# VeeraKarthick609/ImageCaptioner

Measured on NVIDIA B200. Metric: kd_train_samples_per_sec, higher is better.
Workload: dtype bf16

## Files before the change

### imagecaptioner_b200/csrc/api.cu

```cuda
#include <stdlib.h>
#include "gemm.cuh"
#include "loss_kernels.cuh"
#include "decoder_kernels.cuh"
#include "recurrent.cuh"
#include "recur_cluster.cuh"
#include "refine_kernels.cuh"
#include "mha_mma.cuh"
#include "optim_kernels.cuh"

using namespace b2c;

namespace {

constexpr int MAXL = B2C_MAX_LAYERS;
constexpr int COLSUM_RS = 160;

int check_device() {
  static int cached = 1;
  if (cached <= 0) return cached;
  int dev = 0;
  B2C_CUDA(cudaGetDevice(&dev));
  int major = 0;
  B2C_CUDA(cudaDeviceGetAttribute(&major, cudaDevAttrComputeCapabilityMajor, dev));
  if (major != 10) { cached = B2C_EARCH; return set_err(B2C_EARCH, "b2c kernels are built for sm_100a only; device has compute capability major %d", major); }
  cached = 0;
  return 0;
}

struct Carver {
  unsigned char* base; size_t off;
  template <typename U> U* take(size_t n) {
    off = align_up(off, 256);
    U* p = base ? reinterpret_cast<U*>(base + off) : reinterpret_cast<U*>((uintptr_t)0);
    off += n * sizeof(U);
    return p;
  }
};

inline int in_dim(const B2CShape& s, int k) { return k == 0 ? s.E : s.H; }

int check_shape(const B2CShape* s) {
  B2C_CHECK_ARG(s != nullptr, "shape is NULL");
  B2C_CHECK_ARG(s->B > 0 && s->T > 0 && s->S > 0 && s->V > 1, "bad shape B=%d T=%d S=%d V=%d", s->B, s->T, s->S, s->V);
  B2C_CHECK_ARG(s->L >= 1 && s->L <= MAXL, "L=%d outside [1,%d]", s->L, MAXL);
  B2C_CHECK_ARG(s->E > 0 && s->E % 8 == 0 && s->H > 0 && s->H % 8 == 0, "E=%d and H=%d must be positive multiples of 8", s->E, s->H);
  B2C_CHECK_ARG((long)s->B * 4 * s->H < 2147483647L && (long)s->B * s->S * s->E < 2147483647L, "B*4H and B*S*E must stay below 2^31 (32-bit index arithmetic in the per-step kernels)");
  return 0;
}

template <typename T> struct Weights {
  T *Wf, *Wh, *Wce, *Wcc, *W1, *W2, *Wih0, *We; T* Wcat[MAXL]; float* bcat[MAXL]; float* bx;
  T* Wuh;
  void carve(Carver& c, const B2CShape& s) {
    Wf = c.take<T>((size_t)s.E * s.E); Wh = c.take<T>((size_t)s.E * s.H);
// ... 72 lines not shown
  int ncl = cdiv(s.B, 32); if (ncl > mx) ncl = mx;
  if (cdiv(s.B, ncl) > CR_RMAX) return 0;
  return ncl;
}

template <typename T> struct TrainWs {
  Weights<T> w;
  float *P, *u; T *emb, *G0, *o1; T* xh[MAXL]; T* gates[MAXL]; float* c[MAXL];
  T* dgates[MAXL]; float* dxh0; float* dxh[MAXL]; float* dc[MAXL]; T* do1; float* dHext; float* ds; T* du; T* dq; T* dP; float* demb; float* partial;
  float *dWx32, *dWe32; T *dWxT, *dWeT; float* partial_side;
  unsigned int* sync;
  float* EP;
  float* evalp;
  T* G0T;
  float* UR;
  size_t bytes;
  void carve(void* base, const B2CShape& s) {
    Carver c{reinterpret_cast<unsigned char*>(base), 0};
    const size_t B = s.B, Tn = s.T, S = s.S, E = s.E, H = s.H, TB = Tn * B;
    w.carve(c, s);
    P = c.take<float>(B * S * E); emb = c.take<T>(TB * E); u = c.take<float>(TB * E); G0 = c.take<T>(TB * 4 * H); o1 = c.take<T>(TB * E);
    for (int k = 0; k < s.L; ++k) {
      xh[k] = c.take<T>((Tn + 1) * B * (in_dim(s, k) + H));
      gates[k] = c.take<T>(TB * 4 * H);
      this->c[k] = c.take<float>((Tn + 1) * B * H);
    }
    for (int k = 0; k < s.L; ++k) {
      dgates[k] = c.take<T>(TB * 4 * H);
      dxh[k] = k == 0 ? nullptr : c.take<float>(TB * 2 * H);
      dc[k] = c.take<float>(B * H);
    }
    dxh0 = c.take<float>(TB * (E + H));
    do1 = c.take<T>(TB * E); dHext = c.take<float>(TB * H); ds = c.take<float>(TB * S);
    du = c.take<T>(TB * E); dq = c.take<T>(B * H); dP = c.take<T>(B * S * E); demb = c.take<float>(TB * E);
    dWx32 = c.take<float>(4 * H * E); dWe32 = c.take<float>(4 * H * E); dWxT = c.take<T>(4 * H * E); dWeT = c.take<T>(4 * H * E);
    size_t mc = (size_t)s.V; if ((size_t)4 * H > mc) mc = 4 * H; if (E > mc) mc = E;
    partial = c.take<float>((size_t)COLSUM_RS * mc); partial_side = c.take<float>((size_t)COLSUM_RS * mc);
    sync = c.take<unsigned int>(128 + 160 * 32);
    EP = c.take<float>(B * S * E);
    evalp = c.take<float>(TB * (size_t)cdiv(s.V, 32) * EVAL_PART_FLOATS);
    G0T = c.take<T>(cluster_shape_ok(s) ? Tn * (size_t)CR_MAX_CLUSTERS * 4 * H * CR_RMAX : 0);
    UR = c.take<float>(B * (E + 4 * H));
    bytes = align_up(c.off, 256);
  }
};

template <typename T> struct DecodeWs {
  Weights<T> w;
  float *P, *u; T *emb, *G0, *o1; T* xh[MAXL]; float* c[MAXL]; float* logits; int64_t* cur; int32_t* done; float* amax_v; int* amax_i;
  size_t bytes;
  void carve(void* base, const B2CShape& s) {
    Carver c{reinterpret_cast<unsigned char*>(base), 0};
    const size_t B = s.B, S = s.S, E = s.E, H = s.H;
    w.carve(c, s);
    P = c.take<float>(B * S * E); emb = c.take<T>(B * E); u = c.take<float>(B * E); G0 = c.take<T>(B * 4 * H); o1 = c.take<T>(B * E);
    for (int k = 0; k < s.L; ++k) { xh[k] = c.take<T>(2 * B * (in_dim(s, k) + H)); this->c[k] = c.take<float>(B * H); }
    logits = c.take<float>(B * (size_t)s.V); cur = c.take<int64_t>(B); done = c.take<int32_t>(B);
// ... 3 lines not shown
};


template <typename T, typename TC>
int gemm(cudaStream_t st, int M, int N, int K, const T* A, long lda, int a_mn, const T* B, long ldb, int b_mn,
         TC* C, long ldc, float beta, const float* bias, int relu, float alpha, int row_unperm_h) {
  GemmArgs g{M, N, K, alpha, beta, A, lda, a_mn, B, ldb, b_mn, C, ldc, bias, relu};
  g.row_unperm_h = row_unperm_h;
  return Gemm<T, TC>::run(g, st);
}
template <typename T>
int gemm_lstm(cudaStream_t st, int M, int H, int K, const T* A, long lda, const T* Wcat, long ldb, const LstmEpi& le) {
  GemmArgs g{M, 4 * H, K, 1.f, 0.f, A, lda, 0, Wcat, ldb, 0, nullptr, 4 * H, nullptr, 0};
  g.lstm = &le;
  return Gemm<T, float>::run(g, st);
}

inline int ew_grid(long n) { long g = (n + 255) / 256; if (g > 148 * 8) g = 148 * 8; if (g < 1) g = 1; return (int)g; }

template <typename T>
int colsum(cudaStream_t st, const T* A, long rows, int cols, long ld, float* partial, float* out, float* out2 = nullptr, int unperm_h = 0) {
  if (ld == cols && cols % 8 == 0 && ((uintptr_t)A & 15) == 0 && rows >= 256) {
    const int gx = cdiv(cols, 256);
    int rs = (int)((rows + 31) / 32); if (rs > 592 / gx) rs = 592 / gx; if (rs > COLSUM_RS) rs = COLSUM_RS; if (rs < 1) rs = 1;
    colsum_vec_kernel<T, false><<<dim3(gx, rs), 256, 0, st>>>(const_cast<T*>(A), (const T*)nullptr, rows, cols, 1.f, partial);
    B2C_LAUNCH_CHECK("colsum_vec_kernel");
    colsum_final_kernel<<<cdiv(cols, 256), 256, 0, st>>>(partial, rs, cols, out, out2, unperm_h);
    B2C_LAUNCH_CHECK("colsum_final_kernel");
    return 0;
  }
// ... 291 lines not shown

inline int bg_ctas() { static int v = -1; if (v < 0) { const char* e = getenv("B2C_BG_CTAS"); v = e ? atoi(e) : 10; } return v; }
inline bool attn_post_occ3() { static int v = -1; if (v < 0) { const char* e = getenv("B2C_POST_OCC3"); v = (e && e[0] == '0') ? 0 : 1; } return v != 0; }
inline int wgrad_chunks() { static int v = -1; if (v < 0) { const char* e = getenv("B2C_WGRAD_CHUNKS"); v = e ? atoi(e) : 0; } return v; }

template <typename T>
int decoder_backward_impl(const B2CShape& s, const B2CParams& p, const T* feats, const int64_t* cap, const T* hid_top,
                          const float* attw, const T* dlogits, const T* dhid, const B2CGrads& g, float* dfeats,
                          void* ws, size_t ws_bytes, const B2CDropout& dr, cudaStream_t st, int flags) {
  TrainWs<T> W; W.carve(ws, s);
  B2C_CHECK_ARG(ws_bytes >= W.bytes, "workspace too small: %zu < %zu", ws_bytes, W.bytes);
  B2C_CHECK_ARG(g.embedding && g.attn_w && g.attn_b && g.comb_w && g.comb_b && g.out0_w && g.out0_b && g.out3_w && g.out3_b && dfeats, "NULL gradient pointer");
  const int B = s.B, Tn = s.T, S = s.S, E = s.E, H = s.H, L = s.L, V = s.V;
  const long TB = (long)Tn * B;
  const float inv_keep = dr.p > 0.f ? 1.0f / (1.0f - dr.p) : 1.0f;
  SubStreams* hs = nullptr;
  B2C_TRY(get_substreams(&hs));
  cudaStream_t side = hs->s[MAX_SUB - 1];
  for (int k = 0; k < L; ++k) B2C_CHECK_ARG(g.w_ih[k] && g.w_hh[k] && g.b_ih[k] && g.b_hh[k], "NULL LSTM gradient pointer (layer %d)", k);
  B2C_CUDA(cudaEventRecord(hs->ev[3], st));
  B2C_CUDA(cudaStreamWaitEvent(side, hs->ev[3], 0));
  B2C_CUDA(cudaMemsetAsync(W.dxh0, 0, (size_t)TB * (E + H) * sizeof(float), side));
  for (int k = 1; k < L; ++k) B2C_CUDA(cudaMemsetAsync(W.dxh[k], 0, (size_t)TB * 2 * H * sizeof(float), side));
  B2C_CUDA(cudaEventRecord(hs->ev[3], side));
  B2C_TRY((gemm<T, T>(st, (int)TB, E, V, dlogits, V, 0, W.w.W2, E, 1, W.do1, E)));
  relu_bwd_inplace_kernel<T><<<ew_grid(TB * E), 256, 0, st>>>(W.do1, W.o1, TB * E, inv_keep);
  B2C_LAUNCH_CHECK("relu_bwd_inplace_kernel");
  B2C_CUDA(cudaEventRecord(hs->fork, st));
  B2C_CUDA(cudaStreamWaitEvent(side, hs->fork, 0));
  {
    GemmCapScope bg(bg_ctas());
    B2C_TRY((gemm<T, float>(side, V, E, (int)TB, dlogits, V, 1, W.o1, E, 1, g.out3_w, E)));
    B2C_TRY(colsum<T>(side, dlogits, TB, V, V, W.partial_side, g.out3_b));
    B2C_TRY((gemm<T, float>(side, E, H, (int)TB, W.do1, E, 1, hid_top, H, 1, g.out0_w, H)));
    B2C_TRY(colsum<T>(side, W.do1, TB, E, E, W.partial_side, g.out0_b));
  }
  B2C_CUDA(cudaEventRecord(hs->join[MAX_SUB - 1], side));
  B2C_TRY((gemm<T, float>(st, (int)TB, H, E, W.do1, E, 0, W.w.W1, H, 1, W.dHext, H)));
// ... 12 lines not shown
    B2C_TRY((gemm<T, float>(s2, 4 * H, H, K, W.dgates[0] + r0 * 4 * H, 4 * H, 1, W.xh[0] + r0 * (E + H) + E, E + H, 1, g.w_hh[0], H, beta, nullptr, 0, 1.f, H)));
    return 0;
  };
  const int n_chunks = (sp.ns == 1 && bg_ctas() > 0) ? wgrad_chunks() : 0;
  const int chunk_steps = n_chunks > 0 ? cdiv(Tn, n_chunks) : 0;
  long wg_done_from = TB;
  bool wg_any = false;
  pdl_full_dependency_next();
  for (int t = Tn - 1; t >= 0; --t) {
    const bool last = (t == Tn - 1);
    for (int i = 0; i < sp.ns; ++i) {
      cudaStream_t ss = sp.st[i];
      const long b0 = sp.b0[i];
      const int Bh = sp.bn[i];
      const long row = (long)t * B + b0;
      for (int k = L - 1; k >= 0; --k) {
        const int in = in_dim(s, k), ld = in + H;
        const float* carry = last ? nullptr : (k == 0 ? W.dxh0 + (row + B) * (E + H) + E : W.dxh[k] + (row + B) * 2 * H + H);
        const float* above = (k < L - 1) ? W.dxh[k + 1] + row * 2 * H : nullptr;
        const bool top = (k == L - 1);
        B2C_CUDA(launch_pdl(lstm_pointwise_bwd_kernel<T>, dim3(ew_grid((long)Bh * H)), dim3(256), 0, ss,
            (const T*)(W.gates[k] + row * 4 * H), (const float*)(W.c[k] + row * H), (const float*)(W.c[k] + (row + B) * H), W.dc[k] + b0 * H, last ? 1 : 0,
            carry, (long)ld, above, (long)(2 * H), (const float*)(top ? W.dHext + row * H : nullptr), (const T*)((top && dhid) ? dhid + row * H : nullptr),
            (const T*)((top && !last) ? W.dq + b0 * H : nullptr), (long)H, W.dgates[k] + row * 4 * H, Bh, H, dr.p, dr.seed, (uint32_t)k, row, (const unsigned long long*)dr.seed_dev));
        B2C_LAUNCH_CHECK("lstm_pointwise_bwd_kernel");
        float* out = (k == 0) ? W.dxh0 + row * (E + H) : W.dxh[k] + row * 2 * H;
        B2C_TRY((gemm<T, float>(ss, Bh, ld, 4 * H, W.dgates[k] + row * 4 * H, 4 * H, 0, W.w.Wcat[k], ld, 1, out, ld, 1.f)));
      }
      const float* dctx_t = W.dxh0 + row * (E + H);
      T* du_t = W.du + row * E;
      B2C_TRY(attn_bwd<T>(ss, Bh, S, E, W.P + b0 * S * E, feats + b0 * S * E, W.u + row * E, attw + row * S, dctx_t, (long)(E + H), W.ds + row * S, du_t));
      if (t > 0) B2C_TRY((gemm<T, T>(ss, Bh, H, E, du_t, E, 0, W.w.Wh, H, 1, W.dq + b0 * H, H)));
    }
    if (chunk_steps > 0 && t > 0 && (Tn - t) % chunk_steps == 0 && t >= chunk_steps) {
      B2C_CUDA(cudaEventRecord(hs->ev[0], st));
      B2C_CUDA(cudaStreamWaitEvent(side, hs->ev[0], 0));
      GemmCapScope bg(bg_ctas());
      B2C_TRY(weight_grads(side, (long)t * B, wg_done_from, wg_any ? 1.f : 0.f));
      wg_done_from = (long)t * B; wg_any = true;
    }
  }
  B2C_TRY(join_subs(sp));
  B2C_CUDA(cudaEventRecord(hs->ev[1], st));
  B2C_CUDA(cudaStreamWaitEvent(side, hs->ev[1], 0));
  B2C_TRY(weight_grads(side, 0, wg_done_from, wg_any ? 1.f : 0.f));
  for (int k = 0; k < L; ++k) B2C_TRY(colsum<T>(side, W.dgates[k], TB, 4 * H, 4 * H, W.partial_side, g.b_ih[k], g.b_hh[k], H));
  {
// ... 767 lines not shown
```

### imagecaptioner_b200/csrc/gemm.cuh

```cuda
#pragma once
#include "common.cuh"

namespace b2c {

struct LstmEpi {
  int enabled, H;
  const void* addend;
  const float* bias;
  const float* c_prev; float* c_out;
  void* gates_out;
  void* h_rec; long ld_rec; void* h_next; long ld_next; void* h_top; long ld_top;
  float drop_p; unsigned long long seed; unsigned int site; long row_base;
  const unsigned long long* seed_dev;
  const float* addend32; long ld_addend32;
};

constexpr int EVAL_PART_FLOATS = 8;
struct EvalEpi { const float* teacher; const int64_t* targets; float* parts; float inv_temp; int nparts; int cols_per_part; };

struct ArgmaxEpi { float* pmax; int* pidx; int nparts; int cols_per_part; };
inline LstmEpi pack_argmax(const ArgmaxEpi& a) {
  LstmEpi le{};
  le.enabled = 2; le.H = a.nparts; le.c_out = a.pmax; le.gates_out = a.pidx; le.ld_rec = a.cols_per_part;
  return le;
}
inline LstmEpi pack_eval(const EvalEpi& e) {
  LstmEpi le{};
  le.enabled = 3; le.H = e.nparts; le.c_out = e.parts; le.addend = e.teacher; le.h_rec = const_cast<int64_t*>(e.targets);
  le.ld_rec = e.cols_per_part; le.drop_p = e.inv_temp;
  return le;
}

template <typename TL>
__device__ __forceinline__ void lstm_cell_unit(const float (&pre)[4], float c_prev, float (&act)[4], float& c, float& h) {
  act[0] = Math<TL>::sigmoid_(pre[0]); act[1] = Math<TL>::sigmoid_(pre[1]);
  act[2] = Math<TL>::tanh_(pre[2]);    act[3] = Math<TL>::sigmoid_(pre[3]);
  c = fmaf(act[1], c_prev, act[0] * act[2]);
  h = act[3] * Math<TL>::tanh_(c);
}

constexpr int SG_BM = 64, SG_BN = 64, SG_BK = 16;

template <typename TA, typename TB, typename TC>
__global__ void __launch_bounds__(256)
gemm_simt_kernel(int M, int N, int K, float alpha, const TA* __restrict__ A, long lda, int a_mn,
// ... 276 lines not shown
            const uint64_t bdesc = B_MN ? make_smem_desc(sb + k * 2048, 8192, 1024) : make_smem_desc(sb + k * 32, 16, 1024);
            tc_mma_bf16(tacc, adesc, bdesc, idesc, (kb > kb_begin || k > 0) ? 1u : 0u);
          }
          tc_commit(&empty_bar[s]);
        }
        tc_commit(&tfull_bar[as]);
      }
    }
  } else {
    const int q = warp & 3;
    const int half = (warp - 2) >> 2;
    unsigned char* my = epi_stage + (size_t)(warp - 2) * 32 * TC_EPI_PITCH;
    constexpr int PER = 16 / (int)sizeof(TC);
    constexpr int CH = 128 / (int)sizeof(TC);
    const bool vec_ok = (((uintptr_t)C) % 16 == 0) && ((ldc * (long)sizeof(TC)) % 16 == 0);
    int t = 0;
    for (int w = blockIdx.x; w < total; w += gridDim.x, ++t) {
    const int sp = w / tiles_mn, rem = w - sp * tiles_mn;
    const int m0 = (rem / tiles_n) * TC_BM, n0 = (rem % tiles_n) * BN;
    const int as = t & 1; const uint32_t aph = (t >> 1) & 1;
    const bool add_bias = (bias != nullptr) && (sp == 0);
    [[maybe_unused]] float4 pre_b[8]; [[maybe_unused]] uint4 pre_a[4]; [[maybe_unused]] float4 pre_c0, pre_c1; [[maybe_unused]] float4 pre_r[8];
    [[maybe_unused]] int pre_ci = -1;
    if constexpr (LSTM) {
      constexpr int NC32 = BN / 32, C32_PER = (NC32 + 1) / 2;
      const int ci = half * C32_PER, col0 = n0 + ci * 32, grow = m0 + q * 32 + lane;
      if (ci < NC32 && col0 < N && grow < M) {
        pre_ci = ci;
        if (le.bias) {
#pragma unroll
          for (int j = 0; j < 8; ++j) pre_b[j] = *reinterpret_cast<const float4*>(le.bias + col0 + 4 * j);
        }
        if (le.addend) {
          const uint4* ap = reinterpret_cast<const uint4*>(reinterpret_cast<const bf16*>(le.addend) + (long)grow * N + col0);
#pragma unroll
          for (int j = 0; j < 4; ++j) pre_a[j] = ap[j];
        }
        if (le.addend32) {
          const float4* rp = reinterpret_cast<const float4*>(le.addend32 + (long)grow * le.ld_addend32 + col0);
#pragma unroll
          for (int j = 0; j < 8; ++j) pre_r[j] = __ldcg(rp + j);
        }
        pre_c0 = *reinterpret_cast<const float4*>(le.c_prev + (long)grow * le.H + (col0 >> 2));
        pre_c1 = *reinterpret_cast<const float4*>(le.c_prev + (long)grow * le.H + (col0 >> 2) + 4);
      }
    }
    mbar_wait(&tfull_bar[as], aph);
    tc_fence_after();
    const uint32_t tacc = tmem_base + (uint32_t)(as * BN) + ((uint32_t)(q * 32) << 16);
    if constexpr (LSTM) {
      const int H = le.H, N4 = N;
      const int grow = m0 + q * 32 + lane;
      [[maybe_unused]] const float inv_keep = (LSTM_DROP && le.drop_p > 0.f) ? 1.0f / (1.0f - le.drop_p) : 1.0f;
      [[maybe_unused]] const uint64_t dseed = (LSTM_DROP && le.drop_p > 0.f) ? drop_seed(le.seed, le.seed_dev) : 0;
      constexpr int NC32 = BN / 32, C32_PER = (NC32 + 1) / 2;
#pragma unroll 1
      for (int ci = half * C32_PER; ci < (half + 1) * C32_PER && ci < NC32; ++ci) {
        const int col0 = n0 + ci * 32;
        if (col0 >= N) break;
        float v[32];
// ... 157 lines not shown
            for (int j = 0; j < 32; ++j) v[j] = fmaf(alpha, v[j], (bias != nullptr && colb + j < N) ? bias[colb + j] : 0.f);
          }
#pragma unroll
          for (int j = 0; j < 32; ++j) if (colb + j < N && v[j] > best) { best = v[j]; bidx = colb + j; }
        }
      }
      if (grow < M) {
        const int part = (n0 + half * C_PER * CH) / (C_PER * CH);
        if (part < nparts) { pmax[(long)grow * nparts + part] = best; pidx[(long)grow * nparts + part] = bidx; }
      }
      tc_fence_before();
      __syncwarp();
      if (lane == 0) mbar_arrive(&tempty_bar[as]);
      continue;
    }
    if constexpr (EPI == 0 || EPI == 4) {
    if (EPI == 4 || ((split ? sizeof(TC) == 4 : beta == 0.f) && vec_ok && m0 + TC_BM <= M && n0 + BN <= N && (((uintptr_t)bias) & 15) == 0)) {
#pragma unroll 1
      for (int ci = half * C_PER; ci < (half + 1) * C_PER && ci < NCHUNK; ++ci) {
        const int c0 = ci * CH;
#pragma unroll
        for (int h = 0; h < CH / 32; ++h) {
          float v[32];
          tmem_ld32(tacc + (uint32_t)(c0 + h * 32), v);
          if (add_bias) {
            const float4* b4 = reinterpret_cast<const float4*>(bias + n0 + c0 + h * 32);
#pragma unroll
            for (int j = 0; j < 8; ++j) {
              const float4 bb = __ldg(b4 + j);
              v[4 * j] = fmaf(alpha, v[4 * j], bb.x); v[4 * j + 1] = fmaf(alpha, v[4 * j + 1], bb.y);
              v[4 * j + 2] = fmaf(alpha, v[4 * j + 2], bb.z); v[4 * j + 3] = fmaf(alpha, v[4 * j + 3], bb.w);
// ... 24 lines not shown
          const long orow = row_unperm_h ? (long)(grow & 3) * row_unperm_h + (grow >> 2) : (long)grow;
          TC* cp = C + orow * ldc + n0 + c0 + (lane & 7) * PER;
          const uint4 acc = *reinterpret_cast<const uint4*>(my + r * TC_EPI_PITCH + (lane & 7) * 16);
          if (split) {
            asm volatile("red.global.add.v4.f32 [%0], {%1, %2, %3, %4};" :: "l"(cp), "f"(__uint_as_float(acc.x)), "f"(__uint_as_float(acc.y)),
                         "f"(__uint_as_float(acc.z)), "f"(__uint_as_float(acc.w)) : "memory");
          } else {
            *reinterpret_cast<uint4*>(cp) = acc;
          }
        }
        __syncwarp();
      }
      tc_fence_before();
      __syncwarp();
      if (lane == 0) mbar_arrive(&tempty_bar[as]);
      continue;
    }
    if constexpr (EPI == 0) {
#pragma unroll 1
    for (int ci = half * C_PER; ci < (half + 1) * C_PER && ci < NCHUNK; ++ci) {
      const int c0 = ci * CH;
      if (n0 + c0 >= N) break;
#pragma unroll
      for (int h = 0; h < CH / 32; ++h) {
        float v[32];
        tmem_ld32(tacc + (uint32_t)(c0 + h * 32), v);
        const int colb = n0 + c0 + h * 32;
#pragma unroll
        for (int j = 0; j < 32; ++j) {
          float x = alpha * v[j];
          if (add_bias && colb + j < N) x += bias[colb + j];
          if (relu) x = fmaxf(x, 0.f);
          v[j] = x;
// ... 40 lines not shown
            for (int e = 0; e < PER; ++e) {
              if (gcol + e < N) {
                float x = to_f<TC>(a[e]);
                if (beta != 0.f) x += beta * to_f<TC>(cp[e]);
                cp[e] = from_f<TC>(x);
              }
            }
          }
        }
      }
      __syncwarp();
    }
    tc_fence_before();
    __syncwarp();
    if (lane == 0) mbar_arrive(&tempty_bar[as]);
    }
    }
    }
    }
  }
  tc_fence_before();
  __syncthreads();
  if (warp == 1) {
    __syncwarp();
    asm volatile("tcgen05.dealloc.cta_group::1.sync.aligned.b32 %0, %1;" :: "r"(tmem_base), "r"(Cfg::TMEM_COLS) : "memory");
  }
}

typedef CUresult (*PFN_encodeTiled)(CUtensorMap*, CUtensorMapDataType, cuuint32_t, void*, const cuuint64_t*, const cuuint64_t*,
                                    const cuuint32_t*, const cuuint32_t*, CUtensorMapInterleave, CUtensorMapSwizzle,
// ... 24 lines not shown
  if (r != CUDA_SUCCESS) return set_err(B2C_ECUDA, "cuTensorMapEncodeTiled failed (%d): ptr=%p inner=%ld outer=%ld ld=%ld box=%d", (int)r, ptr, inner, outer, ld, box_outer);
  return 0;
}

struct GemmArgs {
  int M, N, K;
  float alpha, beta;
  const void* A; long lda; int a_mn;
  const void* B; long ldb; int b_mn;
  void* C; long ldc;
  const float* bias; int relu;
  int row_unperm_h = 0;
  const LstmEpi* lstm = nullptr;
  ArgmaxEpi* amax = nullptr;
  EvalEpi* eval = nullptr;
};

inline bool tc_eligible(const GemmArgs& g) {
  return ((uintptr_t)g.A % 16 == 0) && ((uintptr_t)g.B % 16 == 0) && (g.lda % 8 == 0) && (g.ldb % 8 == 0);
}

struct TcPlan { int bn, splits, kb_per_split; };
inline TcPlan plan_tc(const GemmArgs& g, int elem_c, int sms) {
  const int num_kb = cdiv(g.K, TC_BK);
  const bool can_split = (elem_c == 4) && !g.relu && (g.beta == 0.f || g.beta == 1.f) && (g.lstm == nullptr) && (g.amax == nullptr) && (g.eval == nullptr);
  TcPlan best{64, 1, num_kb}; double best_cost = 1e30;
  const int cand[3] = {256, 128, 64};
  for (int ci = 0; ci < 3; ++ci) {
    const int bn = cand[ci];
    if (bn > 64 && g.N <= bn / 2) continue;
    const long tiles = (long)cdiv(g.M, TC_BM) * cdiv(g.N, bn);
    int splits = 1;
    if (can_split && tiles < 2L * sms && num_kb >= 16) {
      splits = (int)((2L * sms) / tiles); if (splits > num_kb / 8) splits = num_kb / 8; if (splits < 1) splits = 1;
    }
    const int kbs = cdiv(num_kb, splits); splits = cdiv(num_kb, kbs);
    const long items = tiles * splits;
    const long waves = (items + sms - 1) / sms;
    const double cost = (double)waves * ((double)kbs * (128 + bn) + 6.0 * (128 + bn) + (splits > 1 ? 2.0 : 1.0) * bn * 4.0);
    if (cost < best_cost) { best_cost = cost; best = TcPlan{bn, splits, kbs}; }
// ... 10 lines not shown

inline int& gemm_cta_cap() { static thread_local int c = 0; return c; }
struct GemmCapScope {
  int saved;
  explicit GemmCapScope(int cap) : saved(gemm_cta_cap()) { gemm_cta_cap() = cap; }
  ~GemmCapScope() { gemm_cta_cap() = saved; }
};
inline int gemm_sms() { const int n = sm_count(), c = gemm_cta_cap(); return (c > 0 && c < n) ? c : n; }

template <int BN, bool A_MN, bool B_MN, typename TC>
int launch_tc(const GemmArgs& g, const TcPlan& plan, cudaStream_t st) {
  CUtensorMap ta, tb;
  if (!A_MN) B2C_TRY(make_tmap_bf16(&ta, g.A, g.K, g.M, g.lda, TC_BM)); else B2C_TRY(make_tmap_bf16(&ta, g.A, g.M, g.K, g.lda, 64));
  if (!B_MN) B2C_TRY(make_tmap_bf16(&tb, g.B, g.K, g.N, g.ldb, BN)); else B2C_TRY(make_tmap_bf16(&tb, g.B, g.N, g.K, g.ldb, 64));
  constexpr bool CAN_LSTM = !A_MN && !B_MN && sizeof(TC) == 4;
  void (*kern)(const CUtensorMap, const CUtensorMap, int, int, int, float, float, TC*, long, const float*, int, int, int, int, int, int, const LstmEpi) =
      gemm_tc_kernel<BN, A_MN, B_MN, TC, 0>;
  int flavour = g.lstm ? ((g.lstm->drop_p > 0.f && g.lstm->h_next) ? 1 : 5) : (g.amax ? 2 : (g.eval ? 3 : 0));
  if (flavour == 0 && fast_only_enabled() && g.M % TC_BM == 0 && g.N % BN == 0 && (plan.splits > 1 ? sizeof(TC) == 4 : g.beta == 0.f) &&
      ((uintptr_t)g.C) % 16 == 0 && (g.ldc * (long)sizeof(TC)) % 16 == 0 && (((uintptr_t)g.bias) & 15) == 0) {
    flavour = 4;
    kern = gemm_tc_kernel<BN, A_MN, B_MN, TC, 4>;
  }
  if (flavour != 0 && flavour != 4) {
    if constexpr (CAN_LSTM) {
      kern = flavour == 1 ? gemm_tc_kernel<BN, A_MN, B_MN, TC, 1> : (flavour == 5 ? gemm_tc_kernel<BN, A_MN, B_MN, TC, 5> :
             (flavour == 2 ? gemm_tc_kernel<BN, A_MN, B_MN, TC, 2> : gemm_tc_kernel<BN, A_MN, B_MN, TC, 3>));
    } else return set_err(B2C_EINVAL, "the fused LSTM / argmax / validation epilogues need K-major operands and the fp32 instantiation");
  }
  static bool attr_set[6] = {false, false, false, false, false, false};
  if (!attr_set[flavour]) {
    B2C_CUDA(cudaFuncSetAttribute(kern, cudaFuncAttributeMaxDynamicSharedMemorySize, (int)TcCfg<BN>::SMEM_BYTES));
    attr_set[flavour] = true;
  }
  const int kb_per_split = plan.kb_per_split, splits = plan.splits;
  if (splits > 1 && g.beta == 0.f)
    B2C_CUDA(cudaMemset2DAsync(g.C, (size_t)g.ldc * sizeof(TC), 0, (size_t)g.N * sizeof(TC), (size_t)g.M, st));
  const int tiles_m = cdiv(g.M, TC_BM), tiles_n = cdiv(g.N, BN);
  const long total = (long)tiles_m * tiles_n * splits;
  const int grid = (int)(total < gemm_sms() ? total : gemm_sms());
  LstmEpi epi = g.lstm ? *g.lstm : LstmEpi{};
  if (g.amax) {
    B2C_CHECK_ARG(!g.lstm && splits == 1 && g.amax->pmax && g.amax->pidx, "argmax epilogue: no K split, no LSTM epilogue, partial buffers required");
    constexpr int CHc = 128 / (int)sizeof(TC), CPER = (BN / CHc + 1) / 2;
    g.amax->cols_per_part = CPER * CHc;
    g.amax->nparts = cdiv(g.N, g.amax->cols_per_part);
    epi = pack_argmax(*g.amax);
  }
  if (g.eval) {
    B2C_CHECK_ARG(!g.lstm && !g.amax && splits == 1 && g.eval->teacher && g.eval->targets && g.eval->parts, "validation epilogue: no K split, no other epilogue, buffers required");
    constexpr int CHc = 128 / (int)sizeof(TC), CPER = (BN / CHc + 1) / 2;
    g.eval->cols_per_part = CPER * CHc;
    g.eval->nparts = cdiv(g.N, g.eval->cols_per_part);
    epi = pack_eval(*g.eval);
  }
  B2C_CUDA(launch_pdl(kern, dim3(grid), dim3(TC_THREADS), TcCfg<BN>::SMEM_BYTES, st, ta, tb, g.M, g.N, g.K, g.alpha, g.beta, (TC*)g.C, g.ldc,
                      g.bias, g.relu, kb_per_split, tiles_m, tiles_n, splits, g.row_unperm_h, epi));
  B2C_LAUNCH_CHECK("gemm_tc_kernel");
  return 0;
}

template <int BN, typename TC>
int launch_tc_major(const GemmArgs& g, const TcPlan& plan, cudaStream_t st) {
  if (!g.a_mn && !g.b_mn) return launch_tc<BN, false, false, TC>(g, plan, st);
  if (!g.a_mn && g.b_mn) return launch_tc<BN, false, true, TC>(g, plan, st);
  if (g.a_mn && g.b_mn) return launch_tc<BN, true, true, TC>(g, plan, st);
  return launch_tc<BN, true, false, TC>(g, plan, st);
}

template <typename TC>
int gemm_bf16_tc(const GemmArgs& g, cudaStream_t st) {
  const TcPlan plan = plan_tc(g, (int)sizeof(TC), gemm_sms());
  if (plan.bn == 256) return launch_tc_major<256, TC>(g, plan, st);
  if (plan.bn == 128) return launch_tc_major<128, TC>(g, plan, st);
  return launch_tc_major<64, TC>(g, plan, st);
}

template <typename TA, typename TB, typename TC>
int gemm_simt(const GemmArgs& g, cudaStream_t st) {
  dim3 grid(cdiv(g.N, SG_BN), cdiv(g.M, SG_BM));
  B2C_CUDA(launch_pdl(gemm_simt_kernel<TA, TB, TC>, grid, dim3(256), 0, st, g.M, g.N, g.K, g.alpha, (const TA*)g.A, g.lda, g.a_mn,
                      (const TB*)g.B, g.ldb, g.b_mn, g.beta, (TC*)g.C, g.ldc, g.bias, g.relu, g.row_unperm_h, g.lstm ? *g.lstm : LstmEpi{}));
  B2C_LAUNCH_CHECK("gemm_simt_kernel");
  return 0;
}

template <typename T, typename TC> struct Gemm;
template <typename TC> struct Gemm<float, TC> {
  static int run(const GemmArgs& g, cudaStream_t st) { return gemm_simt<float, float, TC>(g, st); }
};
template <typename TC> struct Gemm<bf16, TC> {
  static int run(const GemmArgs& g, cudaStream_t st) {
    if (tc_eligible(g)) return gemm_bf16_tc<TC>(g, st);
    return gemm_simt<bf16, bf16, TC>(g, st);
// ... 5 lines not shown
```

Before: 208,300.

## Fuse LSTM backward pointwise cell adjoint into recurrent gradient GEMM epilogues

In the BPTT loop on the bf16 path, the separate lstm_pointwise_bwd kernel for lower layers and for the top layer is folded into GEMM epilogues. For the top layer, the dq GEMM computes the next step's gate gradients directly. For lower layers, the dxh GEMM uses split-K with per-tile arrival counters so the last CTA runs the cell adjoint. This removes one kernel launch and one round trip through dq/dxh per layer per timestep. In exchange it adds atomic counters, a memset, heavier epilogues with extra register pressure, and a serialized fixup done by the last-arriving CTA.

```diff
diff --git a/imagecaptioner_b200/csrc/api.cu b/imagecaptioner_b200/csrc/api.cu
--- a/imagecaptioner_b200/csrc/api.cu
+++ b/imagecaptioner_b200/csrc/api.cu
@@ -1,4 +1,5 @@
 #include <stdlib.h>
+#include <type_traits>
 #include "gemm.cuh"
 #include "loss_kernels.cuh"
 #include "decoder_kernels.cuh"
@@ -38,6 +39,9 @@
 };
 
 inline int in_dim(const B2CShape& s, int k) { return k == 0 ? s.E : s.H; }
+constexpr int ADJ_MAX_SUBS = 4;
+inline size_t adj_tiles(const B2CShape& s) { return (size_t)cdiv(s.B, TC_BM) * cdiv(2 * s.H, 64); }
+inline size_t adj_counters(const B2CShape& s) { return (size_t)s.T * (s.L - 1) * ADJ_MAX_SUBS * adj_tiles(s); }
 
 int check_shape(const B2CShape* s) {
   B2C_CHECK_ARG(s != nullptr, "shape is NULL");
@@ -140,6 +144,7 @@
   float* evalp;
   T* G0T;
   float* UR;
+  int* arrivals;
   size_t bytes;
   void carve(void* base, const B2CShape& s) {
     Carver c{reinterpret_cast<unsigned char*>(base), 0};
@@ -167,6 +172,7 @@
     evalp = c.take<float>(TB * (size_t)cdiv(s.V, 32) * EVAL_PART_FLOATS);
     G0T = c.take<T>(cluster_shape_ok(s) ? Tn * (size_t)CR_MAX_CLUSTERS * 4 * H * CR_RMAX : 0);
     UR = c.take<float>(B * (E + 4 * H));
+    arrivals = c.take<int>(adj_counters(s));
     bytes = align_up(c.off, 256);
   }
 };
@@ -200,6 +206,11 @@
   GemmArgs g{M, 4 * H, K, 1.f, 0.f, A, lda, 0, Wcat, ldb, 0, nullptr, 4 * H, nullptr, 0};
   g.lstm = &le;
   return Gemm<T, float>::run(g, st);
+}
+inline int gemm_adj(cudaStream_t st, int M, int N, int K, const bf16* A, long lda, const bf16* W, long ldw, float* C, long ldc, const AdjEpi& a) {
+  GemmArgs g{M, N, K, 1.f, a.fixup ? 1.f : 0.f, A, lda, 0, W, ldw, 1, C, ldc, nullptr, 0};
+  g.adj = &a;
+  return Gemm<bf16, float>::run(g, st);
 }
 
 inline int ew_grid(long n) { long g = (n + 255) / 256; if (g > 148 * 8) g = 148 * 8; if (g < 1) g = 1; return (int)g; }
@@ -521,6 +532,7 @@
   const int B = s.B, Tn = s.T, S = s.S, E = s.E, H = s.H, L = s.L, V = s.V;
   const long TB = (long)Tn * B;
   const float inv_keep = dr.p > 0.f ? 1.0f / (1.0f - dr.p) : 1.0f;
+  constexpr bool FUSED = std::is_same<T, bf16>::value;
   SubStreams* hs = nullptr;
   B2C_TRY(get_substreams(&hs));
   cudaStream_t side = hs->s[MAX_SUB - 1];
@@ -529,6 +541,7 @@
   B2C_CUDA(cudaStreamWaitEvent(side, hs->ev[3], 0));
   B2C_CUDA(cudaMemsetAsync(W.dxh0, 0, (size_t)TB * (E + H) * sizeof(float), side));
   for (int k = 1; k < L; ++k) B2C_CUDA(cudaMemsetAsync(W.dxh[k], 0, (size_t)TB * 2 * H * sizeof(float), side));
+  if (FUSED && L > 1) B2C_CUDA(cudaMemsetAsync(W.arrivals, 0, adj_counters(s) * sizeof(int), side));
   B2C_CUDA(cudaEventRecord(hs->ev[3], side));
   B2C_TRY((gemm<T, T>(st, (int)TB, E, V, dlogits, V, 0, W.w.W2, E, 1, W.do1, E)));
   relu_bwd_inplace_kernel<T><<<ew_grid(TB * E), 256, 0, st>>>(W.do1, W.o1, TB * E, inv_keep);
@@ -571,23 +584,48 @@
       const long b0 = sp.b0[i];
       const int Bh = sp.bn[i];
       const long row = (long)t * B + b0;
+      auto cell_adj = [&](int k, long row, bool lastc) -> AdjEpi {
+        const int ld = in_dim(s, k) + H;
+        const bool top = (k == L - 1);
+        AdjEpi a{};
+        a.H = H; a.gates = (const bf16*)(W.gates[k] + row * 4 * H); a.c_prev = W.c[k] + row * H; a.c_cur = W.c[k] + (row + B) * H;
+        a.dc = W.dc[k] + b0 * H; a.dc_is_zero = lastc ? 1 : 0;
+        a.carry = lastc ? nullptr : (k == 0 ? W.dxh0 + (row + B) * (E + H) + E : W.dxh[k] + (row + B) * 2 * H + H); a.ld_carry = ld;
+        a.ext = top ? W.dHext + row * H : nullptr; a.hid = (const bf16*)((top && dhid) ? dhid + row * H : nullptr);
+        a.dgates = (bf16*)(W.dgates[k] + row * 4 * H);
+        a.drop_p = dr.p; a.seed = dr.seed; a.site = (unsigned)k; a.row_base = row; a.seed_dev = (const unsigned long long*)dr.seed_dev;
+        return a;
+      };
       for (int k = L - 1; k >= 0; --k) {
         const int in = in_dim(s, k), ld = in + H;
-        const float* carry = last ? nullptr : (k == 0 ? W.dxh0 + (row + B) * (E + H) + E : W.dxh[k] + (row + B) * 2 * H + H);
-        const float* above = (k < L - 1) ? W.dxh[k + 1] + row * 2 * H : nullptr;
-        const bool top = (k == L - 1);
-        B2C_CUDA(launch_pdl(lstm_pointwise_bwd_kernel<T>, dim3(ew_grid((long)Bh * H)), dim3(256), 0, ss,
-            (const T*)(W.gates[k] + row * 4 * H), (const float*)(W.c[k] + row * H), (const float*)(W.c[k] + (row + B) * H), W.dc[k] + b0 * H, last ? 1 : 0,
-            carry, (long)ld, above, (long)(2 * H), (const float*)(top ? W.dHext + row * H : nullptr), (const T*)((top && dhid) ? dhid + row * H : nullptr),
-            (const T*)((top && !last) ? W.dq + b0 * H : nullptr), (long)H, W.dgates[k] + row * 4 * H, Bh, H, dr.p, dr.seed, (uint32_t)k, row, (const unsigned long long*)dr.seed_dev));
-        B2C_LAUNCH_CHECK("lstm_pointwise_bwd_kernel");
+        if (!FUSED || (last && k == L - 1)) {
+          const AdjEpi a = cell_adj(k, row, last);
+          const float* above = (k < L - 1) ? W.dxh[k + 1] + row * 2 * H : nullptr;
+          B2C_CUDA(launch_pdl(lstm_pointwise_bwd_kernel<T>, dim3(ew_grid((long)Bh * H)), dim3(256), 0, ss,
+              (const T*)(W.gates[k] + row * 4 * H), a.c_prev, a.c_cur, a.dc, a.dc_is_zero, a.carry, a.ld_carry, above, (long)(2 * H), a.ext,
+              (const T*)((k == L - 1 && dhid) ? dhid + row * H : nullptr), (const T*)((k == L - 1 && !last) ? W.dq + b0 * H : nullptr), (long)H,
+              W.dgates[k] + row * 4 * H, Bh, H, dr.p, dr.seed, (uint32_t)k, row, (const unsigned long long*)dr.seed_dev));
+          B2C_LAUNCH_CHECK("lstm_pointwise_bwd_kernel");
+        }
         float* out = (k == 0) ? W.dxh0 + row * (E + H) : W.dxh[k] + row * 2 * H;
+        if constexpr (FUSED) {
+          if (k > 0) {
+            AdjEpi a = cell_adj(k - 1, row, last);
+            a.fixup = 1;
+            a.arrivals = W.arrivals + (((size_t)t * (L - 1) + (k - 1)) * ADJ_MAX_SUBS + i) * adj_tiles(s);
+            B2C_TRY(gemm_adj(ss, Bh, ld, 4 * H, W.dgates[k] + row * 4 * H, 4 * H, W.w.Wcat[k], ld, out, ld, a));
+            continue;
+          }
+        }
         B2C_TRY((gemm<T, float>(ss, Bh, ld, 4 * H, W.dgates[k] + row * 4 * H, 4 * H, 0, W.w.Wcat[k], ld, 1, out, ld, 1.f)));
       }
       const float* dctx_t = W.dxh0 + row * (E + H);
       T* du_t = W.du + row * E;
       B2C_TRY(attn_bwd<T>(ss, Bh, S, E, W.P + b0 * S * E, feats + b0 * S * E, W.u + row * E, attw + row * S, dctx_t, (long)(E + H), W.ds + row * S, du_t));
-      if (t > 0) B2C_TRY((gemm<T, T>(ss, Bh, H, E, du_t, E, 0, W.w.Wh, H, 1, W.dq + b0 * H, H)));
+      if (t > 0) {
+        if constexpr (FUSED) B2C_TRY(gemm_adj(ss, Bh, H, E, du_t, E, W.w.Wh, H, nullptr, H, cell_adj(L - 1, row - B, false)));
+        else B2C_TRY((gemm<T, T>(ss, Bh, H, E, du_t, E, 0, W.w.Wh, H, 1, W.dq + b0 * H, H)));
+      }
     }
     if (chunk_steps > 0 && t > 0 && (Tn - t) % chunk_steps == 0 && t >= chunk_steps) {
       B2C_CUDA(cudaEventRecord(hs->ev[0], st));
diff --git a/imagecaptioner_b200/csrc/gemm.cuh b/imagecaptioner_b200/csrc/gemm.cuh
--- a/imagecaptioner_b200/csrc/gemm.cuh
+++ b/imagecaptioner_b200/csrc/gemm.cuh
@@ -29,6 +29,99 @@
   le.enabled = 3; le.H = e.nparts; le.c_out = e.parts; le.addend = e.teacher; le.h_rec = const_cast<int64_t*>(e.targets);
   le.ld_rec = e.cols_per_part; le.drop_p = e.inv_temp;
   return le;
+}
+
+struct AdjEpi {
+  int H;
+  const bf16* gates;
+  const float* c_prev; const float* c_cur;
+  float* dc; int dc_is_zero;
+  const float* carry; long ld_carry;
+  const float* ext; const bf16* hid;
+  bf16* dgates;
+  float drop_p; unsigned long long seed; unsigned int site; long row_base; const unsigned long long* seed_dev;
+  int* arrivals;
+  int fixup;
+};
+inline LstmEpi pack_adj(const AdjEpi& a) {
+  LstmEpi le{};
+  le.enabled = a.fixup ? 7 : 6; le.H = a.H;
+  le.addend = a.gates; le.c_prev = a.c_prev; le.bias = a.c_cur; le.c_out = a.dc; le.ld_next = a.dc_is_zero;
+  le.h_rec = const_cast<float*>(a.carry); le.ld_rec = a.ld_carry; le.addend32 = a.ext; le.h_top = const_cast<bf16*>(a.hid);
+  le.gates_out = a.dgates; le.h_next = a.arrivals;
+  le.drop_p = a.drop_p; le.seed = a.seed; le.site = a.site; le.row_base = a.row_base; le.seed_dev = a.seed_dev;
+  return le;
+}
+
+struct Adj8 { uint4 g[4]; float tc[8], cp[8], dh[8], dc[8]; };
+__device__ __forceinline__ void adj_load8(const LstmEpi& le, long r, int u0, Adj8& a) {
+  const int H = le.H;
+  const long e = r * H + u0;
+  const uint4* gp = reinterpret_cast<const uint4*>(reinterpret_cast<const bf16*>(le.addend) + r * 4 * H + 4 * u0);
+#pragma unroll
+  for (int j = 0; j < 4; ++j) a.g[j] = gp[j];
+  const float4 c0 = *reinterpret_cast<const float4*>(le.bias + e), c1 = *reinterpret_cast<const float4*>(le.bias + e + 4);
+  const float4 p0 = *reinterpret_cast<const float4*>(le.c_prev + e), p1 = *reinterpret_cast<const float4*>(le.c_prev + e + 4);
+  const float cc[8] = {c0.x, c0.y, c0.z, c0.w, c1.x, c1.y, c1.z, c1.w};
+  const float cp[8] = {p0.x, p0.y, p0.z, p0.w, p1.x, p1.y, p1.z, p1.w};
+  float4 d0 = make_float4(0.f, 0.f, 0.f, 0.f), d1 = d0;
+  if (!le.ld_next) { d0 = __ldcg(reinterpret_cast<const float4*>(le.c_out + e)); d1 = __ldcg(reinterpret_cast<const float4*>(le.c_out + e + 4)); }
+  const float dc[8] = {d0.x, d0.y, d0.z, d0.w, d1.x, d1.y, d1.z, d1.w};
+  float ext[8] = {0.f, 0.f, 0.f, 0.f, 0.f, 0.f, 0.f, 0.f}, hid[8] = {0.f, 0.f, 0.f, 0.f, 0.f, 0.f, 0.f, 0.f};
+  if (le.addend32) {
+    const float4 x0 = *reinterpret_cast<const float4*>(le.addend32 + e), x1 = *reinterpret_cast<const float4*>(le.addend32 + e + 4);
+    ext[0] = x0.x; ext[1] = x0.y; ext[2] = x0.z; ext[3] = x0.w; ext[4] = x1.x; ext[5] = x1.y; ext[6] = x1.z; ext[7] = x1.w;
+  }
+  if (le.h_top) {
+    const uint4 hv = *reinterpret_cast<const uint4*>(reinterpret_cast<const bf16*>(le.h_top) + e);
+    hid[0] = bf16_lo(hv.x); hid[1] = bf16_hi(hv.x); hid[2] = bf16_lo(hv.y); hid[3] = bf16_hi(hv.y);
+    hid[4] = bf16_lo(hv.z); hid[5] = bf16_hi(hv.z); hid[6] = bf16_lo(hv.w); hid[7] = bf16_hi(hv.w);
+  }
+#pragma unroll
+  for (int u = 0; u < 8; ++u) {
+    a.tc[u] = Math<bf16>::tanh_(cc[u]); a.cp[u] = cp[u]; a.dc[u] = dc[u];
+    float d = 0.f;
+    if (le.addend32) d += ext[u];
+    if (le.h_top) d += hid[u];
+    a.dh[u] = d;
+  }
+}
+template <bool ABOVE>
+__device__ __forceinline__ void adj_finish8(const LstmEpi& le, long r, int u0, Adj8& a, const float* x, uint64_t dseed, float inv_keep) {
+  const int H = le.H;
+  if (le.h_rec) {
+    const float* cp = reinterpret_cast<const float*>(le.h_rec) + r * le.ld_rec + u0;
+    const float4 k0 = __ldcg(reinterpret_cast<const float4*>(cp)), k1 = __ldcg(reinterpret_cast<const float4*>(cp + 4));
+    const float k[8] = {k0.x, k0.y, k0.z, k0.w, k1.x, k1.y, k1.z, k1.w};
+#pragma unroll
+    for (int u = 0; u < 8; ++u) a.dh[u] += k[u];
+  }
+#pragma unroll
+  for (int u = 0; u < 8; ++u) {
+    if (ABOVE) {
+      const float m = le.drop_p > 0.f ? dropout_scale(dseed, le.site, (uint64_t)((le.row_base + r) * H + u0 + u), le.drop_p, inv_keep) : 1.0f;
+      a.dh[u] += x[u] * m;
+    } else {
+      a.dh[u] += to_f<bf16>(from_f<bf16>(x[u]));
+    }
+  }
+  uint32_t dg[16]; float dcn[8];
+#pragma unroll
+  for (int u = 0; u < 8; ++u) {
+    const uint4 gq = a.g[u >> 1];
+    const uint32_t lo = (u & 1) ? gq.z : gq.x, hi = (u & 1) ? gq.w : gq.y;
+    const float i = bf16_lo(lo), f = bf16_hi(lo), g = bf16_lo(hi), o = bf16_hi(hi), tc = a.tc[u], dh = a.dh[u];
+    const float dcc = a.dc[u] + dh * o * (1.0f - tc * tc);
+    dg[2 * u] = pack_bf16(dcc * g * i * (1.0f - i), dcc * a.cp[u] * f * (1.0f - f));
+    dg[2 * u + 1] = pack_bf16(dcc * i * (1.0f - g * g), dh * tc * o * (1.0f - o));
+    dcn[u] = dcc * f;
+  }
+  uint4* gp = reinterpret_cast<uint4*>(reinterpret_cast<bf16*>(le.gates_out) + r * 4 * H + 4 * u0);
+#pragma unroll
+  for (int j = 0; j < 4; ++j) gp[j] = make_uint4(dg[4 * j], dg[4 * j + 1], dg[4 * j + 2], dg[4 * j + 3]);
+  float* dcp = le.c_out + r * H + u0;
+  *reinterpret_cast<float4*>(dcp) = make_float4(dcn[0], dcn[1], dcn[2], dcn[3]);
+  *reinterpret_cast<float4*>(dcp + 4) = make_float4(dcn[4], dcn[5], dcn[6], dcn[7]);
 }
 
 template <typename TL>
@@ -335,6 +428,34 @@
     constexpr int PER = 16 / (int)sizeof(TC);
     constexpr int CH = 128 / (int)sizeof(TC);
     const bool vec_ok = (((uintptr_t)C) % 16 == 0) && ((ldc * (long)sizeof(TC)) % 16 == 0);
+    [[maybe_unused]] auto adj_fixup = [&](int m0, int n0, int rem) {
+      const int H = le.H;
+      if (n0 >= H) return;
+      volatile int* last = reinterpret_cast<volatile int*>(tmem_slot + 1);
+      __threadfence();
+      asm volatile("bar.sync 1, %0;" :: "r"(TC_EPI_WARPS * 32) : "memory");
+      if (warp == 2 && lane == 0) *last = (atomicAdd(reinterpret_cast<int*>(le.h_next) + rem, 1) == splits - 1);
+      asm volatile("bar.sync 1, %0;" :: "r"(TC_EPI_WARPS * 32) : "memory");
+      if (!*last) return;
+      __threadfence();
+      const int grow = m0 + q * 32 + lane;
+      if (grow >= M) return;
+      const float inv_keep = le.drop_p > 0.f ? 1.0f / (1.0f - le.drop_p) : 1.0f;
+      const uint64_t dseed = le.drop_p > 0.f ? drop_seed(le.seed, le.seed_dev) : 0;
+      constexpr int NC32 = BN / 32, C32_PER = (NC32 + 1) / 2;
+#pragma unroll 1
+      for (int ci = half * C32_PER; ci < (half + 1) * C32_PER && ci < NC32; ++ci) {
+#pragma unroll 1
+        for (int u0 = n0 + ci * 32; u0 < n0 + ci * 32 + 32 && u0 < H; u0 += 8) {
+          Adj8 a;
+          adj_load8(le, grow, u0, a);
+          const float* cp = reinterpret_cast<const float*>(C) + (long)grow * ldc + u0;
+          const float4 x0 = __ldcg(reinterpret_cast<const float4*>(cp)), x1 = __ldcg(reinterpret_cast<const float4*>(cp + 4));
+          const float x[8] = {x0.x, x0.y, x0.z, x0.w, x1.x, x1.y, x1.z, x1.w};
+          adj_finish8<true>(le, grow, u0, a, x, dseed, inv_keep);
+        }
+      }
+    };
     int t = 0;
     for (int w = blockIdx.x; w < total; w += gridDim.x, ++t) {
     const int sp = w / tiles_mn, rem = w - sp * tiles_mn;
@@ -365,6 +486,11 @@
         pre_c0 = *reinterpret_cast<const float4*>(le.c_prev + (long)grow * le.H + (col0 >> 2));
         pre_c1 = *reinterpret_cast<const float4*>(le.c_prev + (long)grow * le.H + (col0 >> 2) + 4);
       }
+    }
+    [[maybe_unused]] Adj8 pre_adj;
+    if constexpr (EPI == 6) {
+      const int col0 = n0 + half * ((BN / 32 + 1) / 2) * 32, grow = m0 + q * 32 + lane;
+      if (grow < M && col0 < N) adj_load8(le, grow, col0, pre_adj);
     }
     mbar_wait(&tfull_bar[as], aph);
     tc_fence_after();
@@ -552,7 +678,36 @@
       if (lane == 0) mbar_arrive(&tempty_bar[as]);
       continue;
     }
-    if constexpr (EPI == 0 || EPI == 4) {
+    if constexpr (EPI == 6) {
+      constexpr int NC32 = BN / 32, C32_PER = (NC32 + 1) / 2;
+      const int grow = m0 + q * 32 + lane;
+#pragma unroll 1
+      for (int ci = half * C32_PER; ci < (half + 1) * C32_PER && ci < NC32; ++ci) {
+        const int col0 = n0 + ci * 32;
+        if (col0 >= N) break;
+        float v[32];
+        tmem_ld32(tacc + (uint32_t)(ci * 32), v);
+        if (grow < M) {
+#pragma unroll
+          for (int g = 0; g < 4; ++g) {
+            const int u0 = col0 + 8 * g;
+            if (u0 >= N) break;
+            if (g == 0 && ci == half * C32_PER) {
+              adj_finish8<false>(le, grow, u0, pre_adj, v, 0, 1.f);
+            } else {
+              Adj8 a;
+              adj_load8(le, grow, u0, a);
+              adj_finish8<false>(le, grow, u0, a, v + 8 * g, 0, 1.f);
+            }
+          }
+        }
+      }
+      tc_fence_before();
+      __syncwarp();
+      if (lane == 0) mbar_arrive(&tempty_bar[as]);
+      continue;
+    }
+    if constexpr (EPI == 0 || EPI == 4 || EPI == 7) {
     if (EPI == 4 || ((split ? sizeof(TC) == 4 : beta == 0.f) && vec_ok && m0 + TC_BM <= M && n0 + BN <= N && (((uintptr_t)bias) & 15) == 0)) {
 #pragma unroll 1
       for (int ci = half * C_PER; ci < (half + 1) * C_PER && ci < NCHUNK; ++ci) {
@@ -607,9 +762,10 @@
       tc_fence_before();
       __syncwarp();
       if (lane == 0) mbar_arrive(&tempty_bar[as]);
+      if constexpr (EPI == 7) adj_fixup(m0, n0, rem);
       continue;
     }
-    if constexpr (EPI == 0) {
+    if constexpr (EPI == 0 || EPI == 7) {
 #pragma unroll 1
     for (int ci = half * C_PER; ci < (half + 1) * C_PER && ci < NCHUNK; ++ci) {
       const int c0 = ci * CH;
@@ -680,6 +836,7 @@
     tc_fence_before();
     __syncwarp();
     if (lane == 0) mbar_arrive(&tempty_bar[as]);
+    if constexpr (EPI == 7) adj_fixup(m0, n0, rem);
     }
     }
     }
@@ -734,8 +891,10 @@
   const LstmEpi* lstm = nullptr;
   ArgmaxEpi* amax = nullptr;
   EvalEpi* eval = nullptr;
+  const AdjEpi* adj = nullptr;
 };
 
+inline bool vec_ok_c(const GemmArgs& g) { return ((uintptr_t)g.C % 16 == 0) && ((g.ldc * 4) % 16 == 0); }
 inline bool tc_eligible(const GemmArgs& g) {
   return ((uintptr_t)g.A % 16 == 0) && ((uintptr_t)g.B % 16 == 0) && (g.lda % 8 == 0) && (g.ldb % 8 == 0);
 }
@@ -743,7 +902,8 @@
 struct TcPlan { int bn, splits, kb_per_split; };
 inline TcPlan plan_tc(const GemmArgs& g, int elem_c, int sms) {
   const int num_kb = cdiv(g.K, TC_BK);
-  const bool can_split = (elem_c == 4) && !g.relu && (g.beta == 0.f || g.beta == 1.f) && (g.lstm == nullptr) && (g.amax == nullptr) && (g.eval == nullptr);
+  const bool can_split = (elem_c == 4) && !g.relu && (g.beta == 0.f || g.beta == 1.f) && (g.lstm == nullptr) && (g.amax == nullptr) && (g.eval == nullptr) &&
+                         (g.adj == nullptr || g.adj->fixup);
   TcPlan best{64, 1, num_kb}; double best_cost = 1e30;
   const int cand[3] = {256, 128, 64};
   for (int ci = 0; ci < 3; ++ci) {
@@ -784,21 +944,26 @@
   if (!A_MN) B2C_TRY(make_tmap_bf16(&ta, g.A, g.K, g.M, g.lda, TC_BM)); else B2C_TRY(make_tmap_bf16(&ta, g.A, g.M, g.K, g.lda, 64));
   if (!B_MN) B2C_TRY(make_tmap_bf16(&tb, g.B, g.K, g.N, g.ldb, BN)); else B2C_TRY(make_tmap_bf16(&tb, g.B, g.N, g.K, g.ldb, 64));
   constexpr bool CAN_LSTM = !A_MN && !B_MN && sizeof(TC) == 4;
+  constexpr bool CAN_ADJ = !A_MN && B_MN && sizeof(TC) == 4;
   void (*kern)(const CUtensorMap, const CUtensorMap, int, int, int, float, float, TC*, long, const float*, int, int, int, int, int, int, const LstmEpi) =
       gemm_tc_kernel<BN, A_MN, B_MN, TC, 0>;
-  int flavour = g.lstm ? ((g.lstm->drop_p > 0.f && g.lstm->h_next) ? 1 : 5) : (g.amax ? 2 : (g.eval ? 3 : 0));
+  int flavour = g.lstm ? ((g.lstm->drop_p > 0.f && g.lstm->h_next) ? 1 : 5) : (g.amax ? 2 : (g.eval ? 3 : (g.adj ? (g.adj->fixup ? 7 : 6) : 0)));
   if (flavour == 0 && fast_only_enabled() && g.M % TC_BM == 0 && g.N % BN == 0 && (plan.splits > 1 ? sizeof(TC) == 4 : g.beta == 0.f) &&
       ((uintptr_t)g.C) % 16 == 0 && (g.ldc * (long)sizeof(TC)) % 16 == 0 && (((uintptr_t)g.bias) & 15) == 0) {
     flavour = 4;
     kern = gemm_tc_kernel<BN, A_MN, B_MN, TC, 4>;
   }
-  if (flavour != 0 && flavour != 4) {
+  if (flavour == 6 || flavour == 7) {
+    if constexpr (CAN_ADJ) {
+      kern = flavour == 6 ? gemm_tc_kernel<BN, A_MN, B_MN, TC, 6> : gemm_tc_kernel<BN, A_MN, B_MN, TC, 7>;
+    } else return set_err(B2C_EINVAL, "the fused cell-adjoint epilogue needs a K-major A, an MN-major B and the fp32 instantiation");
+  } else if (flavour != 0 && flavour != 4) {
     if constexpr (CAN_LSTM) {
       kern = flavour == 1 ? gemm_tc_kernel<BN, A_MN, B_MN, TC, 1> : (flavour == 5 ? gemm_tc_kernel<BN, A_MN, B_MN, TC, 5> :
              (flavour == 2 ? gemm_tc_kernel<BN, A_MN, B_MN, TC, 2> : gemm_tc_kernel<BN, A_MN, B_MN, TC, 3>));
     } else return set_err(B2C_EINVAL, "the fused LSTM / argmax / validation epilogues need K-major operands and the fp32 instantiation");
   }
-  static bool attr_set[6] = {false, false, false, false, false, false};
+  static bool attr_set[8] = {false, false, false, false, false, false, false, false};
   if (!attr_set[flavour]) {
     B2C_CUDA(cudaFuncSetAttribute(kern, cudaFuncAttributeMaxDynamicSharedMemorySize, (int)TcCfg<BN>::SMEM_BYTES));
     attr_set[flavour] = true;
@@ -824,6 +989,14 @@
     g.eval->nparts = cdiv(g.N, g.eval->cols_per_part);
     epi = pack_eval(*g.eval);
   }
+  if (g.adj) {
+    const AdjEpi& a = *g.adj;
+    B2C_CHECK_ARG(!g.lstm && !g.amax && !g.eval && a.H % 8 == 0 && a.gates && a.c_prev && a.c_cur && a.dc && a.dgates,
+                  "cell-adjoint epilogue: no other epilogue, H a multiple of 8, saved operands required");
+    if (a.fixup) B2C_CHECK_ARG(g.beta == 1.f && g.C && vec_ok_c(g) && a.H <= g.N && a.arrivals, "cell-adjoint fixup: zeroed fp32 C (beta = 1), 16-byte rows, arrival counters required");
+    else B2C_CHECK_ARG(splits == 1 && g.N == a.H && !a.arrivals, "cell-adjoint epilogue of the top layer: N == H, no K split");
+    epi = pack_adj(a);
+  }
   B2C_CUDA(launch_pdl(kern, dim3(grid), dim3(TC_THREADS), TcCfg<BN>::SMEM_BYTES, st, ta, tb, g.M, g.N, g.K, g.alpha, g.beta, (TC*)g.C, g.ldc,
                       g.bias, g.relu, kb_per_split, tiles_m, tiles_n, splits, g.row_unperm_h, epi));
   B2C_LAUNCH_CHECK("gemm_tc_kernel");
@@ -848,6 +1021,7 @@
 
 template <typename TA, typename TB, typename TC>
 int gemm_simt(const GemmArgs& g, cudaStream_t st) {
+  B2C_CHECK_ARG(!g.adj, "the fused cell-adjoint epilogue exists on the tcgen05 path only");
   dim3 grid(cdiv(g.N, SG_BN), cdiv(g.M, SG_BM));
   B2C_CUDA(launch_pdl(gemm_simt_kernel<TA, TB, TC>, grid, dim3(256), 0, st, g.M, g.N, g.K, g.alpha, (const TA*)g.A, g.lda, g.a_mn,
                       (const TB*)g.B, g.ldb, g.b_mn, g.beta, (TC*)g.C, g.ldc, g.bias, g.relu, g.row_unperm_h, g.lstm ? *g.lstm : LstmEpi{}));
```

Result: slower. 161,000, median of 6 (-22.7%).
